# aaryaamoharir/ImageTransformations

Measured on AMD Instinct MI355X. Metric: Mpixels/sec, 5x5 Gaussian + bilinear rotate on 4K RGB; % HBM roofline, higher is better.
Workload: dtype u8/f32

## Files before the change

imagetransformations_amd/csrc/affine_route.h:

```cpp
#pragma once
#include "imgxf_common.h"
#include <algorithm>
#include <string.h>

namespace imgxf {

struct AffineParams {
    double m[6];
    int fx[6];
    int64_t q0, q3;
    int64_t q1, q4;
    int64_t x00, y00;
    u32 ntx_magic;
    int sx[4], sy[4];
    u8 fill[4];
    int xcd_regions;
};

constexpr int BILINEAR_LIST_MAX = 896;
struct TileList { int n; u32 idx[BILINEAR_LIST_MAX]; };

constexpr int MF_TILE_H = 64;
constexpr int WQ_PITCH = 28;
constexpr int WQ_MAXCH = 192;
constexpr int NQ_KW = 8;
constexpr int TALL_PITCH = 49, TALL_MAXROWS = 64;

struct AffineKnobs {
    bool fpb_set;
    int fpb;
    bool no_dma, no_lds, no_shear_fast, no_tall;
    int fpb_or(int dflt) const { return fpb_set ? fpb : dflt; }
};

enum AffineFamily {
    AF_GLOBAL,
    AF_BILINEAR_GLOBAL,
    AF_BILINEAR_LDS,
    AF_BILINEAR_INTERIOR,
    AF_BILINEAR_LIST,
    AF_BILINEAR_MF,
    AF_BILINEAR_WQ,
    AF_NEAREST_LDS,
    AF_NEAREST_DMA,
    AF_NEAREST_WQ,
    AF_SHEAR,
    AF_SHEAR_EDGES,
};

struct AffineLaunch {
    AffineFamily family;
    int c, filter, pitch, nbr, kw, tile_h;
    bool precise, dbg, dma, honly, defer;
    dim3 grid, block;
    size_t lds;
    int ntx, nty, fpb, nch, bh;
};

struct AffinePlan {
    AffineParams P;
    int n;
    AffineLaunch launch[2];
    TileList list;
};

inline int box_f64(double a, double b, int tw, int th, int extra) {
    return (int)ceil(fabs(a) * (tw - 1) + fabs(b) * (th - 1)) + extra;
}
inline int box_fx(int a, int b, int tw, int th, int extra) {
    return (int)ceil((fabs((double)a) * (tw - 1) + fabs((double)b) * (th - 1)) / 65536.0) + extra;
}
inline int packed_chunks(int bw) { return (bw * 3 + 15 + 15) / 16; }
inline bool aligned(const View& v, int bytes) {
    return ((((uintptr_t)v.p) | (uintptr_t)v.rs | (uintptr_t)v.fs) & (uintptr_t)(bytes - 1)) == 0;
}
inline bool offsets_fit_32(const View& v) { return (int64_t)v.h * v.rs < ((int64_t)1 << 32); }
inline u32 tile_magic(int ntx) { return (u32)((((uint64_t)1 << 32) + ntx - 1) / ntx); }
__host__ __device__ inline bool xcd_tile(unsigned b, int ntx, int nty, int regions, u32 magic, int& tx, int& ty) {
    const int T = ntx * nty, x = (int)(b & 7), l = (int)(b >> 3), q = T >> 3, r = T & 7;
    const int first = x * q + (x < r ? x : r), count = q + (x < r);
    if (l >= count) return false;
    if (!regions) {
        const int t = first + l;
        ty = magic ? (int)(((uint64_t)(u32)t * magic) >> 32) : t / ntx;
        tx = t - ty * ntx;
        return true;
    }
    const int last = first + count - 1;
    const int c0 = first / nty, r0 = first - c0 * nty, c1 = last / nty, r1 = last - c1 * nty;
    if (c1 == c0) { tx = c0; ty = r0 + l; return true; }
    const int whole = c1 - c0 - 1;
    const bool both = r0 <= r1 + 1;
    const int lo = both ? r0 : r1 + 1, hi = both ? r1 + 1 : r0;
    const int w1 = both ? whole + 2 : whole, n0 = lo * (whole + 1), n1 = (hi - lo) * w1;
    if (l < n0) { ty = l / (whole + 1); tx = c0 + 1 + (l - ty * (whole + 1)); }
    else if (l < n0 + n1) { const int k = l - n0, row = k / w1; ty = lo + row; tx = (both ? c0 : c0 + 1) + (k - row * w1); }
    else { const int k = l - n0 - n1, row = k / (whole + 1); ty = hi + row; tx = c0 + (k - row * (whole + 1)); }
    return true;
}
inline unsigned xcd_tile_grid(int ntx, int nty, int min_cols, AffineParams& P) {
    P.xcd_regions = ntx >= min_cols;
    return (unsigned)(ntx * nty);
}

inline AffineLaunch& add_launch(AffinePlan& R, AffineFamily family, dim3 grid, dim3 block, size_t lds) {
    AffineLaunch& L = R.launch[R.n++];
    L = AffineLaunch();
    L.family = family; L.grid = grid; L.block = block; L.lds = lds;
    return L;
}

inline bool plan_nearest_tiles(const View& s, const View& d, const AffineKnobs& K, AffinePlan& R) {
    AffineParams& P = R.P;
    bool nowrap = true;
    for (int cy = 0; cy < 2; ++cy)
        for (int cx = 0; cx < 2; ++cx) {
            const double X = cx ? d.w + 32 : 0, Y = cy ? d.h + 32 : 0;
            const double xs = (double)P.fx[2] + (double)P.fx[1] * Y + (double)P.fx[0] * X;
            const double ys = (double)P.fx[5] + (double)P.fx[4] * Y + (double)P.fx[3] * X;
            if (fabs(xs) > 2.0e9 || fabs(ys) > 2.0e9) nowrap = false;
        }
    const int bw = box_fx(P.fx[0], P.fx[1], 32, 32, 3), bh = box_fx(P.fx[3], P.fx[4], 32, 32, 3);
    const int ntx = (d.w + 31) / 32, nty = (d.h + 31) / 32;
    if (!(nowrap && bw <= 97 && bh <= 100 && (int64_t)ntx * nty < 0x7fffffff && d.n <= 65535)) return false;
    P.ntx_magic = tile_magic(ntx);
    {
        const int bwq = box_fx(P.fx[0], P.fx[1], 32, 16, 3), bhq = box_fx(P.fx[3], P.fx[4], 32, 16, 3);
        const int nchq = packed_chunks(bwq), kwq = (bhq * nchq + 63) / 64;
        const int ntxq = (d.w + 127) / 128, ntyq = (d.h + 15) / 16;
        if (aligned(s, 16) && aligned(d, 16) && (d.w * 3) % 16 == 0 && (s.w * 3) % 16 == 0 && s.w * 3 >= 16 && offsets_fit_32(s) &&
            offsets_fit_32(d) && !K.no_dma && kwq <= NQ_KW && (int64_t)ntxq * ntyq < ((int64_t)1 << 27)) {
            const int fpbq = std::max(1, std::min(K.fpb_or(1), d.n));
            const size_t nbufq = fpbq > 1 ? 2 : 1;
            AffineLaunch& L = add_launch(R, AF_NEAREST_WQ, dim3((unsigned)(ntxq * ntyq), (unsigned)((d.n + fpbq - 1) / fpbq)), dim3(256),
                                         nbufq * ((size_t)4 * ((size_t)bhq * nchq * 16 + 16) + 16 * 384));
            L.kw = kwq; L.ntx = ntxq; L.nty = ntyq; L.fpb = fpbq; L.nch = nchq; L.bh = bhq;
            return true;
        }
    }
    if (bw <= 49 && bh <= 52 && !K.no_dma && s.w * 3 >= 16 && (s.w * 3) % 16 == 0 && aligned(s, 16)) {
        const int bw64 = box_fx(P.fx[0], P.fx[1], 32, 64, 3), bh64 = box_fx(P.fx[3], P.fx[4], 32, 64, 3);
        if (bw64 <= 64 && bh64 <= 80 && !K.no_tall) {
            const int nty64 = (d.h + 63) / 64;
            const unsigned gx = xcd_tile_grid(ntx, nty64, 16, P);
            AffineLaunch& L = add_launch(R, AF_NEAREST_DMA, dim3(gx, (unsigned)d.n), dim3(256), (size_t)13 * 16 * bh64 + 32);
            L.tile_h = 64; L.ntx = ntx; L.nty = nty64;
        } else {
            AffineLaunch& L = add_launch(R, AF_NEAREST_DMA, dim3((unsigned)(ntx * nty), (unsigned)d.n), dim3(256), (size_t)11 * 16 * bh + 32);
            L.tile_h = 32; L.ntx = ntx; L.nty = nty;
        }
        return true;
    }
    const int pitch = bw <= 49 ? 49 : (bw <= 65 ? 65 : 97);
    AffineLaunch& L = add_launch(R, AF_NEAREST_LDS, dim3((unsigned)(ntx * nty), (unsigned)d.n), dim3(256), (size_t)pitch * bh * 4 + 16);
    L.pitch = pitch; L.ntx = ntx; L.nty = nty;
    return true;
}

inline bool plan_fixed_point(const View& d, const double* m, AffineParams& P) {
    bool fixed_ok = fabs(m[0]) < 64.0 && fabs(m[3]) < 64.0;
    for (int cy = 0; cy < 2 && fixed_ok; ++cy)
        for (int cx = 0; cx < 2; ++cx) {
            const double X = (cx ? d.w + 4 : 0) + 0.5, Y = (cy ? d.h : 0) + 0.5;
            const double xs = m[0] * X + m[1] * Y + m[2], ys = m[3] * X + m[4] * Y + m[5];
            if (!(fabs(xs) < 2097152.0 && fabs(ys) < 2097152.0)) fixed_ok = false;
        }
    P.q0 = fixed_ok ? llround(m[0] * 1099511627776.0) : 0;
    P.q3 = fixed_ok ? llround(m[3] * 1099511627776.0) : 0;
    fixed_ok = fixed_ok && fabs(m[1]) < 64.0 && fabs(m[4]) < 64.0;
    P.q1 = fixed_ok ? llround(m[1] * 1099511627776.0) : 0;
    P.q4 = fixed_ok ? llround(m[4] * 1099511627776.0) : 0;
    for (int k = 0; k < 4; ++k) {
        P.sx[k] = (int)((k * P.q0 + (k * P.q0 >= 0 ? 32768 : -32768)) / 65536);
        P.sy[k] = (int)((k * P.q3 + (k * P.q3 >= 0 ? 32768 : -32768)) / 65536);
    }
    if (fixed_ok) {
        const double x0d = (m[0] * 0.5 + m[1] * 0.5) + m[2] - 0.5, y0d = (m[3] * 0.5 + m[4] * 0.5) + m[5] - 0.5;
        P.x00 = (int64_t)floor(x0d * 1099511627776.0);
        P.y00 = (int64_t)floor(y0d * 1099511627776.0);
    }
    return fixed_ok;
}

inline bool plan_bilinear_tall(const View& s, const View& d, const double* m, int bw, int bh, int ntx, bool pr, bool want_f32,
                               const AffineKnobs& K, AffinePlan& R) {
    AffineParams& P = R.P;
    const int bwt = box_f64(m[0], m[1], 32, MF_TILE_H, 4), bht = box_f64(m[3], m[4], 32, MF_TILE_H, 4);
    const int ntyt = (d.h + MF_TILE_H - 1) / MF_TILE_H;
    if (bwt > TALL_PITCH || bht > TALL_MAXROWS || bw > TALL_PITCH || (int64_t)ntx * ntyt * ntx >= ((int64_t)1 << 32)) return false;
    const int fpb = K.fpb_or(16);
    const bool mf = !want_f32 && fpb >= 2 && d.n >= 2 && bht <= 64 && offsets_fit_32(d);
    if (mf && !K.no_dma) {
        const int bwq = box_f64(m[0], m[1], 32, 16, 4), bhq = box_f64(m[3], m[4], 32, 16, 4);
        const int nchq = packed_chunks(bwq);
        const int ntxq = (d.w + 127) / 128, ntyq = (d.h + 15) / 16;
        if (aligned(s, 16) && aligned(d, 16) && (d.w * 3) % 16 == 0 && s.w * 3 >= 16 &&
            bwq <= WQ_PITCH && bhq * nchq <= WQ_MAXCH && bhq * (WQ_PITCH / 4) <= 192 &&
            offsets_fit_32(s) && (int64_t)ntxq * ntyq < ((int64_t)1 << 27)) {
            const int fpbq = K.fpb_or(24);
            const unsigned gx = xcd_tile_grid(ntxq, ntyq, 8, P);
            AffineLaunch& L = add_launch(R, AF_BILINEAR_WQ, dim3(gx, (unsigned)((d.n + fpbq - 1) / fpbq)), dim3(256),
                                         (size_t)4 * ((size_t)bhq * WQ_PITCH * 4 + 2 * ((size_t)bhq * nchq * 16 + 64)) + 2 * 16 * 384);
            L.precise = pr; L.ntx = ntxq; L.nty = ntyq; L.fpb = fpbq; L.nch = nchq; L.bh = bhq;
            return true;
        }
    }
    const int nch = packed_chunks(bwt);
    if (mf && !K.no_dma && bht <= 52 && bwt <= 52 && 52 * nch <= 768 && aligned(s, 16) && s.w * 3 >= 16 && offsets_fit_32(s)) {
        const unsigned gx = xcd_tile_grid(ntx, ntyt, 16, P);
        AffineLaunch& L = add_launch(R, AF_BILINEAR_MF, dim3(gx, (unsigned)((d.n + fpb - 1) / fpb)), dim3(256),
                                     (size_t)52 * 56 * 4 + 2 * ((size_t)52 * nch * 16 + 64));
        L.precise = pr; L.pitch = 56; L.nbr = 13; L.dma = true; L.ntx = ntx; L.nty = ntyt; L.fpb = fpb; L.nch = nch;
        return true;
    }
    struct { int n; u32* idx; } list = {0, R.list.idx};
    const int64_t q0 = P.q0, q1 = P.q1, q3 = P.q3, q4 = P.q4, x00 = P.x00, y00 = P.y00;
    const int sw = s.w, sh = s.h, dw = d.w, dh = d.h;
    const int64_t ax = 31 * q0, bx = (MF_TILE_H - 1) * q1, ay = 31 * q3, by = (MF_TILE_H - 1) * q4;
    const int64_t xlo_o = std::min(ax, (int64_t)0) + std::min(bx, (int64_t)0), xhi_o = std::max(ax, (int64_t)0) + std::max(bx, (int64_t)0);
    const int64_t ylo_o = std::min(ay, (int64_t)0) + std::min(by, (int64_t)0), yhi_o = std::max(ay, (int64_t)0) + std::max(by, (int64_t)0);
    for (int ty = 0; ty < ntyt && list.n <= BILINEAR_LIST_MAX; ++ty)
        for (int tx = 0; tx < ntx; ++tx) {
            const int64_t XT = x00 + (int64_t)(tx * 32) * q0 + (int64_t)(ty * MF_TILE_H) * q1;
            const int64_t YT = y00 + (int64_t)(tx * 32) * q3 + (int64_t)(ty * MF_TILE_H) * q4;
            const bool clean = (int)((XT + xlo_o) >> 40) >= 0 && (int)((YT + ylo_o) >> 40) >= 0 &&
                               (int)((XT + xhi_o) >> 40) + 1 <= sw - 1 && (int)((YT + yhi_o) >> 40) + 1 <= sh - 1 &&
                               tx * 32 + 32 <= dw && ty * MF_TILE_H + MF_TILE_H <= dh &&
                               !((int)((XT + xhi_o) >> 40) + 1 == sw - 1 && (int)((YT + yhi_o) >> 40) + 1 == sh - 1);
            if (!clean) {
                if (list.n < BILINEAR_LIST_MAX) list.idx[list.n] = (u32)(ty * ntx + tx);
                ++list.n;
            }
        }
    R.list.n = list.n;
    if (list.n > BILINEAR_LIST_MAX) return false;
    if (list.n < ntx * ntyt && mf) {
        const int nbr = bht <= 52 ? 13 : 16;
        AffineLaunch& L = add_launch(R, AF_BILINEAR_MF, dim3((unsigned)(ntx * ntyt), (unsigned)((d.n + fpb - 1) / fpb)), dim3(256),
                                     (size_t)2 * TALL_PITCH * (4 * nbr) * 4 + 16);
        L.precise = pr; L.pitch = TALL_PITCH; L.nbr = nbr; L.ntx = ntx; L.nty = ntyt; L.fpb = fpb;
    } else if (list.n < ntx * ntyt) {
        AffineLaunch& L = add_launch(R, AF_BILINEAR_INTERIOR, dim3((unsigned)(ntx * ntyt), (unsigned)d.n), dim3(256),
                                     (size_t)TALL_PITCH * bht * 4 + 16);
        L.precise = pr; L.dbg = want_f32; L.pitch = TALL_PITCH; L.tile_h = MF_TILE_H; L.ntx = ntx; L.nty = ntyt;
    }
    if (list.n > 0) {
        AffineLaunch& L = add_launch(R, AF_BILINEAR_LIST, dim3((unsigned)((MF_TILE_H / 32) * list.n), (unsigned)d.n), dim3(256),
                                     (size_t)TALL_PITCH * bh * 4 + 16);
        L.precise = pr; L.dbg = want_f32; L.pitch = TALL_PITCH; L.tile_h = MF_TILE_H; L.ntx = ntx;
    }
    return true;
}

inline bool plan_bilinear_tiles(const View& s, const View& d, const double* m, bool pr, bool want_f32, const AffineKnobs& K,
                                AffinePlan& R) {
    const int bw = box_f64(m[0], m[1], 32, 32, 4), bh = box_f64(m[3], m[4], 32, 32, 4);
    const int ntx = (d.w + 31) / 32, nty = (d.h + 31) / 32;
    if (!(bw <= 97 && bh <= 100 && (int64_t)ntx * nty < 0x7fffffff && d.n <= 65535)) return false;
    R.P.ntx_magic = tile_magic(ntx);
    if (!K.no_tall && plan_bilinear_tall(s, d, m, bw, bh, ntx, pr, want_f32, K, R)) return true;
    const int pitch = bw <= 49 ? 49 : (bw <= 65 ? 65 : 97);
    AffineLaunch& L = add_launch(R, AF_BILINEAR_LDS, dim3((unsigned)(ntx * nty), (unsigned)d.n), dim3(256), (size_t)pitch * bh * 4 + 16);
    L.precise = pr; L.dbg = want_f32; L.pitch = pitch; L.ntx = ntx; L.nty = nty;
    return true;
}

inline bool horizontal_only(const double* m) {
    return m[3] == 0.0 && m[4] == 1.0 && m[5] == floor(m[5]) && fabs(m[5]) < 1.0e9;
}

inline int plan_affine(const View& s, const View& d, const double* m, int filter, bool precise, bool want_f32, const u8* fill,
                       const AffineKnobs& K, AffinePlan& R) {
    AffineParams& P = R.P;
    memset(&P, 0, sizeof(P));
    for (int i = 0; i < 6; ++i) P.m[i] = m[i];
    affine_fixed_matrix(m, P.fx);
    if (fill) for (int j = 0; j < d.c; ++j) P.fill[j] = fill[j];
    R.n = 0;
    R.list.n = 0;
    const bool pr = precise || filter == IMGXF_FILTER_NEAREST;
    if (filter == IMGXF_FILTER_NEAREST && s.c == 3 && !K.no_lds && aligned(s, 4) && plan_nearest_tiles(s, d, K, R)) return IMGXF_OK;
    const bool fixed_ok = plan_fixed_point(d, m, P);
    if (filter == IMGXF_FILTER_BILINEAR && (s.c == 1 || s.c == 3) && s.w >= 3 && s.h >= 2 && fixed_ok) {
        if (s.c == 3 && !K.no_lds && aligned(s, 4) && plan_bilinear_tiles(s, d, m, pr, want_f32, K, R)) return IMGXF_OK;
        constexpr int BW = 2 * 8 * 4, BH = (4 / 2) * (64 / 8);
        const int ntx = (d.w + BW - 1) / BW, nty = (d.h + BH - 1) / BH;
        const int64_t nb = (int64_t)ntx * nty * d.n;
        if (nb > 0x7fffffff) return IMGXF_ERR_SHAPE;
        AffineLaunch& L = add_launch(R, AF_BILINEAR_GLOBAL, dim3((unsigned)nb), dim3(256), 0);
        L.c = s.c; L.precise = pr; L.ntx = ntx; L.nty = nty;
        return IMGXF_OK;
    }
    const bool honly = horizontal_only(m);
    if (filter == IMGXF_FILTER_BICUBIC && honly && s.c == 3 && !want_f32 && !K.no_shear_fast && s.w >= 4) {
        AffineLaunch& L = add_launch(R, AF_SHEAR, dim3((unsigned)((d.w + 1023) / 1024), (unsigned)d.h, (unsigned)d.n), dim3(256), 0);
        L.precise = pr;
        L.defer = m[0] == 1.0;
        if (L.defer) add_launch(R, AF_SHEAR_EDGES, dim3((unsigned)((d.h * 8 + 255) / 256), (unsigned)d.n), dim3(256), 0);
        return IMGXF_OK;
    }
    AffineLaunch& L = add_launch(R, AF_GLOBAL, dim3((unsigned)((d.w + 255) / 256), (unsigned)((d.h + 3) / 4), (unsigned)d.n), dim3(64, 4), 0);
    L.c = s.c; L.filter = filter; L.precise = pr;
    L.honly = filter == IMGXF_FILTER_BICUBIC && honly;
    return IMGXF_OK;
}

}
```

imagetransformations_amd/csrc/affine_wq.inc:

```
#pragma once

namespace imgxf {


template <int OFF>
__device__ __forceinline__ u32 wq_bytes_at(const u32 (&q)[4]) {
    if constexpr ((OFF & 3) == 0) return q[OFF >> 2];
    else return __builtin_amdgcn_alignbyte(q[(OFF >> 2) + 1], q[OFF >> 2], (u32)(OFF & 3));
}

typedef u32 wq_u32x4 __attribute__((ext_vector_type(4)));

__device__ __forceinline__ void store16_sv(u8* base, u32 voff, wq_u32x4 o) {
    asm volatile("global_store_dwordx4 %0, %1, %2" : : "v"(voff), "v"(o), "s"(base) : "memory");
}

struct WqFlush {
    u32 rd[2], off[2];
    bool ok[2];
    __device__ __forceinline__ WqFlush(const View& d, const u32* slots, int lane, int wave, int txb, int sy0) {
        const int rb16 = (int)((int64_t)d.w * 3 / 16);
#pragma unroll
        for (int pass = 0; pass < 2; ++pass) {
            const int ch = pass * 64 + lane;
            const int r = wave * 4 + ch / 24, ck = ch - (ch / 24) * 24;
            ok[pass] = ch < 96 && sy0 + r < d.h && txb * 24 + ck < rb16;
            rd[pass] = (u32)(uintptr_t)(__attribute__((address_space(3))) const u32*)slots + (u32)((r * 96 + ck * 4) * 4);
            off[pass] = (u32)(sy0 + r) * (u32)d.rs + (u32)(txb * 384 + ck * 16);
        }
    }
    template <u32 SLOT_OFF>
    __device__ __forceinline__ void rows(u8* dframe) const {
#pragma unroll
        for (int pass = 0; pass < 2; ++pass) {
            if (ok[pass]) store16_sv(dframe, off[pass], *(const __attribute__((address_space(3))) wq_u32x4*)(uintptr_t)(rd[pass] + SLOT_OFF));
        }
    }
    __device__ __forceinline__ void operator()(u8* dframe, int par) const {
        if (par) rows<16 * 96 * 4>(dframe); else rows<0>(dframe);
    }
};

template <bool PRECISE>
__global__ __launch_bounds__(256, 3) void affine_bilinear_wq_kernel(View s, View d, AffineParams P, int ntx, int nty, int fpb,
                                                                   int nch, int rows) {
    constexpr int C = 3, SW = 32, BH = 16, BW = 4 * SW, PITCH = WQ_PITCH, NG = PITCH / 4;
    constexpr float GUARDP = 4.0f / 32768.0f;
    constexpr u32 GTOP = 8u << 17;
    constexpr int FONE = 1 << 24, FHALF = 1 << 23, CG32 = 1 << 6;
    extern __shared__ __attribute__((aligned(16))) u32 wq_lds[];
    int tyb, txb;
    if (!xcd_tile(blockIdx.x, ntx, nty, P.xcd_regions, 0, txb, tyb)) return;
    const int lane = threadIdx.x & 63, wave = __builtin_amdgcn_readfirstlane(threadIdx.x >> 6);
    const int f_begin = blockIdx.y * fpb, f_end = min(d.n, f_begin + fpb);
    const int sx0 = txb * BW + wave * SW, sy0 = tyb * BH;
    const bool wave_in = sx0 < d.w;

    const u32 pk_bytes = (u32)(rows * nch * 16 + 64);
    const u32 wave_bytes = (u32)(rows * PITCH * 4) + 2u * pk_bytes;
    u32* const srct = wq_lds + wave * (wave_bytes / 4);
    u32* const slots = wq_lds + 4 * (wave_bytes / 4);

    const int64_t XT = P.x00 + (int64_t)sx0 * P.q0 + (int64_t)sy0 * P.q1;
    const int64_t YT = P.y00 + (int64_t)sx0 * P.q3 + (int64_t)sy0 * P.q4;
    const int64_t ax = (SW - 1) * P.q0, bx = (BH - 1) * P.q1, ay = (SW - 1) * P.q3, by = (BH - 1) * P.q4;
    const int64_t xlo = XT + min(ax, (int64_t)0) + min(bx, (int64_t)0), xhi = XT + max(ax, (int64_t)0) + max(bx, (int64_t)0);
    const int64_t ylo = YT + min(ay, (int64_t)0) + min(by, (int64_t)0), yhi = YT + max(ay, (int64_t)0) + max(by, (int64_t)0);
    const int ux_lo = __builtin_amdgcn_readfirstlane((int)(xlo >> 40)), uy_lo = __builtin_amdgcn_readfirstlane((int)(ylo >> 40));
    const int sx_hi = __builtin_amdgcn_readfirstlane((int)(xhi >> 40) + 1), sy_hi = __builtin_amdgcn_readfirstlane((int)(yhi >> 40) + 1);
    const bool interior = ux_lo >= 0 && uy_lo >= 0 && sx_hi <= s.w - 1 && sy_hi <= s.h - 1 && sx0 + SW <= d.w && sy0 + BH <= d.h;

    const int lx = (lane & 7) * 4, x0 = sx0 + lx;
    u32 la[8];
    float w00[8], w01[8], w10[8], w11[8];
    u32 cneed = 0, fillm = 0, okm = 0;
#pragma unroll
    for (int half = 0; half < 2; ++half) {
        const int ly = half * 8 + (lane >> 3);
        const int64_t XL = XT + lx * P.q0 + ly * P.q1 - ((int64_t)ux_lo << 40);
        const int64_t YL = YT + lx * P.q3 + ly * P.q4 - ((int64_t)uy_lo << 40);
        const int Xb = (int)((XL + 32768) >> 16), Yb = (int)((YL + 32768) >> 16);
#pragma unroll
        for (int j = 0; j < 4; ++j) {
            const int k = half * 4 + j;
            const int X32 = Xb + P.sx[j], Y32 = Yb + P.sy[j];
            const u32 fx = (u32)X32 & (FONE - 1), fy = (u32)Y32 & (FONE - 1);
            const float dx = (float)fx * 5.9604644775390625e-08f, dy = (float)fy * 5.9604644775390625e-08f;
            const float ox = 1.0f - dx, oy = 1.0f - dy;
            w00[k] = ox * oy; w01[k] = dx * oy; w10[k] = ox * dy; w11[k] = dx * dy;
            la[k] = (u32)(((Y32 >> 24) * PITCH + (X32 >> 24)) * 4);
            const u32 gx = ((u32)X32 + CG32) & (FONE - 1), gy = ((u32)Y32 + CG32) & (FONE - 1);
            cneed |= (min(gx, gy) < 2u * CG32) ? 1u << k : 0u;
            if (!interior) {
                const int xi = (X32 >> 24) + ux_lo, yi = (Y32 >> 24) + uy_lo;
                const bool valid = x0 + j < d.w && sy0 + ly < d.h;
                const bool sure = (((fx & (FHALF - 1)) - CG32) < (u32)(FHALF - 2 * CG32)) &&
                                  (((fy & (FHALF - 1)) - CG32) < (u32)(FHALF - 2 * CG32));
                const bool inner = valid && sure && xi >= 0 && xi + 1 <= s.w - 1 && yi >= 0 && yi + 1 <= s.h - 1;
                const bool far_out = valid && sure && (xi < -1 || xi > s.w || yi < -1 || yi > s.h);
                if (!inner) { w00[k] = 0.0f; w01[k] = 0.0f; w10[k] = 0.0f; w11[k] = 0.0f; la[k] = 0u; }
                cneed = (cneed & ~(1u << k)) | ((valid && !inner && !far_out) ? 1u << k : 0u);
                fillm |= far_out ? 1u << k : 0u;
                okm |= valid ? 1u << k : 0u;
            }
        }
    }
    const bool fill_only = wave_in && !interior && __builtin_amdgcn_ballot_w64((okm & ~fillm) != 0u) == 0;
    const bool wave_on = wave_in && !fill_only;
    if (interior) okm = 0xffu;

    const int a0 = (ux_lo * 3) & ~15, e0 = ux_lo * 3 - a0;
    const u32 rgbx_bytes = (u32)(rows * PITCH * 4);
    const u32 pk_base = (u32)(uintptr_t)(__attribute__((address_space(3))) u32*)srct + rgbx_bytes;
    u32 dma_off[3];
    bool dma_ok[3];
    u32 ex_rd[3], ex_wr[3];
    bool ex_ok[3];
    {
        const u32 lim = (u32)(((int64_t)(s.h - 1) * s.rs + (int64_t)s.w * 3 - 16) & ~(int64_t)15);
#pragma unroll
        for (int i = 0; i < 3; ++i) {
            const int c = i * 64 + lane;
            const int row = c / nch, ch = c - row * nch;
            dma_ok[i] = c < rows * nch && wave_on;
            const int64_t go = (int64_t)clampi(uy_lo + row, 0, s.h - 1) * s.rs + a0 + 16 * ch;
            dma_off[i] = (u32)min(max(go, (int64_t)0), (int64_t)lim);
        }
#pragma unroll
        for (int it = 0; it < 3; ++it) {
            const int u = lane + 64 * it;
            const int rr = u / NG, t = u - rr * NG;
            ex_ok[it] = u < rows * NG;
            ex_rd[it] = pk_base + (u32)(rr * nch * 16 + ((e0 + 12 * t) & ~3));
            ex_wr[it] = pk_base - rgbx_bytes + (u32)((rr * PITCH + 4 * t) * 4);
            asm volatile("" : "+v"(ex_rd[it]), "+v"(ex_wr[it]));
        }
    }
    const int kw = (rows * nch + 63) / 64;
    auto dma_issue = [&](const u8* fb, int pbuf) {
#pragma unroll
        for (int i = 0; i < 3; ++i) {
            const u32 ldst = __builtin_amdgcn_readfirstlane(pk_base + (u32)pbuf * pk_bytes + (u32)(i * 1024));
            if (i < kw && dma_ok[i]) glds16_hidden(fb, dma_off[i], ldst);
        }
    };
    auto expand = [&](auto ph, int pbuf) {
        constexpr int PH = decltype(ph)::value;
        const u32 poff = (u32)pbuf * pk_bytes;
#pragma unroll
        for (int it = 0; it < 3; ++it) {
            if (!ex_ok[it]) continue;
            const __attribute__((address_space(3))) u32* q = (const __attribute__((address_space(3))) u32*)(uintptr_t)(ex_rd[it] + poff);
            const u32 dq[4] = {q[0], q[1], q[2], q[3]};
            const wq_u32x4 o = {wq_bytes_at<PH>(dq), wq_bytes_at<PH + 3>(dq), wq_bytes_at<PH + 6>(dq), wq_bytes_at<PH + 9>(dq)};
            *(__attribute__((address_space(3))) wq_u32x4*)(uintptr_t)ex_wr[it] = o;
        }
    };

    auto put_pixel = [&](u32 (&od)[2][3], int k, u32 val) {
        const int half = k >> 2, j = k & 3;
        u32 o0 = half ? od[1][0] : od[0][0], o1 = half ? od[1][1] : od[0][1], o2 = half ? od[1][2] : od[0][2];
        if (j == 0) o0 = (o0 & 0xff000000u) | val;
        else if (j == 1) { o0 = (o0 & 0x00ffffffu) | (val << 24); o1 = (o1 & 0xffff0000u) | (val >> 8); }
        else if (j == 2) { o1 = (o1 & 0x0000ffffu) | (val << 16); o2 = (o2 & 0xffffff00u) | (val >> 16); }
        else o2 = (o2 & 0x000000ffu) | (val << 8);
        if (half) { od[1][0] = o0; od[1][1] = o1; od[1][2] = o2; } else { od[0][0] = o0; od[0][1] = o1; od[0][2] = o2; }
    };

    auto slow_pixels = [&](u32 need, int f, u32 (&od)[2][3]) {
        const u8* sp = s.p + (int64_t)f * s.fs;
#pragma unroll 1
        for (u32 m = need; m; m &= m - 1) {
            const int k = __builtin_ctz(m), half = k >> 2, j = k & 3;
            const int y = sy0 + half * 8 + (lane >> 3);
            const bool unsure = (cneed >> k) & 1u;
            u32 val = 0;
            bool have = true;
            const double xc = (double)(x0 + j) + 0.5, yc = (double)y + 0.5;
            double xin = (P.m[0] * xc + P.m[1] * yc) + P.m[2];
            double yin = (P.m[3] * xc + P.m[4] * yc) + P.m[5];
            if (unsure && !(xin >= 0.0 && xin < (double)s.w && yin >= 0.0 && yin < (double)s.h)) {
                val = (u32)P.fill[0] | ((u32)P.fill[1] << 8) | ((u32)P.fill[2] << 16);
            } else {
                xin -= 0.5; yin -= 0.5;
                const double xfl = floor(xin), yfl = floor(yin);
                const int xq = (int)xfl, yq = (int)yfl;
                const double dxd = xin - xfl, dyd = yin - yfl;
                u32 p00, p01, p10, p11;
                if (unsure) {
                    const int xa = clampi(xq, 0, s.w - 1) * C, xb = clampi(xq + 1, 0, s.w - 1) * C;
                    const u8* r0 = sp + (int64_t)clampi(yq, 0, s.h - 1) * s.rs;
                    const bool has1 = (yq + 1 >= 0) && (yq + 1 < s.h);
                    const u8* r1 = has1 ? sp + (int64_t)(yq + 1) * s.rs : r0;
                    p00 = (u32)r0[xa] | ((u32)r0[xa + 1] << 8) | ((u32)r0[xa + 2] << 16);
                    p01 = (u32)r0[xb] | ((u32)r0[xb + 1] << 8) | ((u32)r0[xb + 2] << 16);
                    p10 = (u32)r1[xa] | ((u32)r1[xa + 1] << 8) | ((u32)r1[xa + 2] << 16);
                    p11 = (u32)r1[xb] | ((u32)r1[xb + 1] << 8) | ((u32)r1[xb + 2] << 16);
                } else {
                    const u32* tp = srct + (yq - uy_lo) * PITCH + (xq - ux_lo);
                    p00 = tp[0]; p01 = tp[1]; p10 = tp[PITCH]; p11 = tp[PITCH + 1];
                    have = (((p00 ^ p01) | (p10 ^ p11) | (p00 ^ p10)) << 8) != 0;
                }
#pragma unroll
                for (int c = 0; c < C; ++c) {
                    const double ta = (double)((p00 >> (8 * c)) & 0xffu), tb = (double)((p01 >> (8 * c)) & 0xffu);
                    const double tc = (double)((p10 >> (8 * c)) & 0xffu), te = (double)((p11 >> (8 * c)) & 0xffu);
                    const double w1 = ta + (tb - ta) * dxd, w2 = tc + (te - tc) * dxd;
                    const double w = w1 + (w2 - w1) * dyd;
                    val |= (u32)(u8)(int)w << (8 * c);
                }
            }
            if (have) put_pixel(od, k, val);
        }
    };

    auto gather_frame = [&](int f, u32* slot) {
        const u32 boff = (u32)(uintptr_t)(__attribute__((address_space(3))) const u32*)srct;
        u32 od[2][3] = {{0u, 0u, 0u}, {0u, 0u, 0u}};
        u32 need = cneed;
#pragma unroll
        for (int half = 0; half < 2; ++half) {
            if (half) __builtin_amdgcn_sched_barrier(0);
            u32 tq[4][3], mq[4];
#pragma unroll
            for (int j = 0; j < 4; ++j) {
                const int k = half * 4 + j;
                const u32* tp = (const u32*)(__attribute__((address_space(3))) const u32*)(uintptr_t)(boff + la[k]);
                const u32 p00 = tp[0], p01 = tp[1], p10 = tp[PITCH], p11 = tp[PITCH + 1];
                constexpr float X0 = PRECISE ? 256.0f + GUARDP : 0.0f;
                float v[3];
                v[0] = fmaf(w00[k], tapf<0>(p00), X0); v[1] = fmaf(w00[k], tapf<1>(p00), X0); v[2] = fmaf(w00[k], tapf<2>(p00), X0);
                v[0] = fmaf(w01[k], tapf<0>(p01), v[0]); v[1] = fmaf(w01[k], tapf<1>(p01), v[1]); v[2] = fmaf(w01[k], tapf<2>(p01), v[2]);
                v[0] = fmaf(w10[k], tapf<0>(p10), v[0]); v[1] = fmaf(w10[k], tapf<1>(p10), v[1]); v[2] = fmaf(w10[k], tapf<2>(p10), v[2]);
                v[0] = fmaf(w11[k], tapf<0>(p11), v[0]); v[1] = fmaf(w11[k], tapf<1>(p11), v[1]); v[2] = fmaf(w11[k], tapf<2>(p11), v[2]);
                if (PRECISE) {
#pragma unroll
                    for (int c = 0; c < 3; ++c) tq[j][c] = __builtin_amdgcn_alignbit(__float_as_uint(v[c]), __float_as_uint(v[c]), 15u);
                    mq[j] = min(min(tq[j][0], tq[j][1]), tq[j][2]);
                } else {
                    u32 (&o)[3] = od[half];
#pragma unroll
                    for (int c = 0; c < 3; ++c) {
                        const int bpos = j * 3 + c;
                        o[bpos >> 2] = __builtin_amdgcn_cvt_pk_u8_f32(floorf(v[c]), bpos & 3, o[bpos >> 2]);
                    }
                }
            }
            if (PRECISE) {
                constexpr u32 PAIR = 0x0c0c0400u, QUAD = 0x05040100u;
                const u32 a0 = __builtin_amdgcn_perm(tq[0][1], tq[0][0], PAIR), a1 = __builtin_amdgcn_perm(tq[1][0], tq[0][2], PAIR);
                const u32 a2 = __builtin_amdgcn_perm(tq[1][2], tq[1][1], PAIR), a3 = __builtin_amdgcn_perm(tq[2][1], tq[2][0], PAIR);
                const u32 a4 = __builtin_amdgcn_perm(tq[3][0], tq[2][2], PAIR), a5 = __builtin_amdgcn_perm(tq[3][2], tq[3][1], PAIR);
                od[half][0] = __builtin_amdgcn_perm(a1, a0, QUAD);
                od[half][1] = __builtin_amdgcn_perm(a3, a2, QUAD);
                od[half][2] = __builtin_amdgcn_perm(a5, a4, QUAD);
                const u32 mg = min(min(mq[0], mq[1]), min(mq[2], mq[3]));
                if (__builtin_amdgcn_ballot_w64(mg < GTOP) != 0) {
#pragma unroll
                    for (int j = 0; j < 4; ++j) need |= (mq[j] < GTOP) ? 1u << (half * 4 + j) : 0u;
                }
            }
        }
        need &= okm & ~fillm;
        if (need) slow_pixels(need, f, od);
        if (fillm && ((u32)P.fill[0] | (u32)P.fill[1] | (u32)P.fill[2])) {
            const u32 val = (u32)P.fill[0] | ((u32)P.fill[1] << 8) | ((u32)P.fill[2] << 16);
#pragma unroll 1
            for (u32 m = fillm; m; m &= m - 1) put_pixel(od, __builtin_ctz(m), val);
        }
#pragma unroll
        for (int half = 0; half < 2; ++half) {
            u32* ws = slot + (half * 8 + (lane >> 3)) * 96 + wave * 24 + (lane & 7) * 3;
            ws[0] = od[half][0]; ws[1] = od[half][1]; ws[2] = od[half][2];
        }
    };

    const WqFlush flush_slot(d, slots, lane, wave, txb, sy0);

    if (fill_only) {
        const u32 val = (u32)P.fill[0] | ((u32)P.fill[1] << 8) | ((u32)P.fill[2] << 16);
#pragma unroll
        for (int q = 0; q < 4; ++q) {
            u32* ws = slots + (q >> 1) * (16 * 96) + ((q & 1) * 8 + (lane >> 3)) * 96 + wave * 24 + (lane & 7) * 3;
            ws[0] = val | (val << 24); ws[1] = (val >> 8) | (val << 16); ws[2] = (val >> 16) | (val << 8);
        }
    }

    const u8* sdma = s.p + (int64_t)f_begin * s.fs;
    u8* dfl = d.p + (int64_t)f_begin * d.fs;
    if (wave_on) {
        dma_issue(sdma, 0); sdma += s.fs;
        if (f_begin + 1 < f_end) { dma_issue(sdma, 1); sdma += s.fs; }
    }
    const int ph = e0 & 3;
    int pb = 0;
#pragma unroll 1
    for (int f = f_begin; f < f_end; ++f) {
        const int par = (f - f_begin) & 1;
        if (wave_on) {
            if (f + 1 >= f_end) asm volatile("s_waitcnt vmcnt(0)" ::: "memory");
            else if (kw == 1) asm volatile("s_waitcnt vmcnt(1)" ::: "memory");
            else if (kw == 2) asm volatile("s_waitcnt vmcnt(2)" ::: "memory");
            else asm volatile("s_waitcnt vmcnt(3)" ::: "memory");
        }
        if (f > f_begin) { flush_slot(dfl, par ^ 1); dfl += d.fs; }
        if (wave_on) {
            if (ph == 0) expand(std::integral_constant<int, 0>(), pb);
            else if (ph == 1) expand(std::integral_constant<int, 1>(), pb);
            else if (ph == 2) expand(std::integral_constant<int, 2>(), pb);
            else expand(std::integral_constant<int, 3>(), pb);
            asm volatile("s_waitcnt lgkmcnt(0)" ::: "memory");
            if (f + 2 < f_end) { dma_issue(sdma, pb); sdma += s.fs; }
            gather_frame(f, slots + par * (16 * 96));
            pb ^= 1;
        }
        asm volatile("s_waitcnt lgkmcnt(0)\n\ts_barrier" ::: "memory");
    }
    flush_slot(dfl, (f_end - 1 - f_begin) & 1);
}


template <int KWT>
__device__ __forceinline__ void nq_wait() {
    static_assert(KWT >= 0 && KWT <= NQ_KW, "");
    if constexpr (KWT == 0) asm volatile("s_waitcnt vmcnt(0)" ::: "memory");
    else if constexpr (KWT == 1) asm volatile("s_waitcnt vmcnt(1)" ::: "memory");
    else if constexpr (KWT == 2) asm volatile("s_waitcnt vmcnt(2)" ::: "memory");
    else if constexpr (KWT == 3) asm volatile("s_waitcnt vmcnt(3)" ::: "memory");
    else if constexpr (KWT == 4) asm volatile("s_waitcnt vmcnt(4)" ::: "memory");
    else if constexpr (KWT == 5) asm volatile("s_waitcnt vmcnt(5)" ::: "memory");
    else if constexpr (KWT == 6) asm volatile("s_waitcnt vmcnt(6)" ::: "memory");
    else if constexpr (KWT == 7) asm volatile("s_waitcnt vmcnt(7)" ::: "memory");
    else asm volatile("s_waitcnt vmcnt(8)" ::: "memory");
}

template <int KW>
__global__ __launch_bounds__(256) void affine_nearest_wq_kernel(View s, View d, AffineParams P, int ntx, int nty, int fpb,
                                                                int nch, int rows) {
    constexpr int C = 3, SW = 32, BH = 16, BW = 4 * SW;
    extern __shared__ __attribute__((aligned(16))) u32 nq_lds[];
    int tyb, txb;
    if (!xcd_tile(blockIdx.x, ntx, nty, P.xcd_regions, 0, txb, tyb)) return;
    const int lane = threadIdx.x & 63, wave = __builtin_amdgcn_readfirstlane(threadIdx.x >> 6);
    const int f_begin = blockIdx.y * fpb, f_end = min(d.n, f_begin + fpb);
    const int sx0 = txb * BW + wave * SW, sy0 = tyb * BH;
    const int dpitch = nch * 16;
    const u32 box_bytes = (u32)(rows * dpitch + 16);
    const u32 nbuf = fpb > 1 ? 2u : 1u;
    char* const boxes = (char*)nq_lds + wave * (nbuf * box_bytes);
    u32* const slots = nq_lds + 4 * (nbuf * box_bytes) / 4;

    const int XT = P.fx[2] + P.fx[1] * sy0 + P.fx[0] * sx0;
    const int YT = P.fx[5] + P.fx[4] * sy0 + P.fx[3] * sx0;
    const int ax = (SW - 1) * P.fx[0], bx = (BH - 1) * P.fx[1], ay = (SW - 1) * P.fx[3], by = (BH - 1) * P.fx[4];
    const int sx_lo = max((XT + min(ax, 0) + min(bx, 0)) >> 16, 0), sx_hi = min((XT + max(ax, 0) + max(bx, 0)) >> 16, s.w - 1);
    const int sy_lo = max((YT + min(ay, 0) + min(by, 0)) >> 16, 0), sy_hi = min((YT + max(ay, 0) + max(by, 0)) >> 16, s.h - 1);
    const int bwc = sx_hi - sx_lo + 1, bhc = sy_hi - sy_lo + 1;
    const bool wave_in = sx0 < d.w && bwc > 0 && bhc > 0;
    const int a0 = (sx_lo * 3) & ~15;
    const int last_chunk = s.w * 3 - 16;

    const u32 fillw = (u32)P.fill[0] | ((u32)P.fill[1] << 8) | ((u32)P.fill[2] << 16);
    const int lx = (lane & 7) * 4;
    u32 bo[8];
    u32 inm = 0;
#pragma unroll
    for (int half = 0; half < 2; ++half) {
        const int ly = half * 8 + (lane >> 3);
        const int XL = XT + lx * P.fx[0] + ly * P.fx[1], YL = YT + lx * P.fx[3] + ly * P.fx[4];
#pragma unroll
        for (int j = 0; j < 4; ++j) {
            const int xi = ((XL + j * P.fx[0]) >> 16) - sx_lo, yi = ((YL + j * P.fx[3]) >> 16) - sy_lo;
            const bool in = wave_in && (u32)xi < (u32)bwc && (u32)yi < (u32)bhc;
            bo[half * 4 + j] = in ? (u32)(yi * dpitch + (xi + sx_lo) * 3 - a0) : 0u;
            inm |= in ? 1u << (half * 4 + j) : 0u;
        }
    }

    u32 dma_off[KW];
    bool dma_ok[KW];
#pragma unroll
    for (int i = 0; i < KW; ++i) {
        const int c = i * 64 + lane;
        const int row = c / nch, ch = c - row * nch;
        dma_ok[i] = wave_in && c < rows * nch;
        dma_off[i] = (u32)((int64_t)min(sy_lo + row, s.h - 1) * s.rs + min(a0 + ch * 16, last_chunk));
    }
    const u32 box_base = (u32)(uintptr_t)(__attribute__((address_space(3))) char*)boxes;
    auto dma_issue = [&](const u8* fb, int pbuf) {
#pragma unroll
        for (int i = 0; i < KW; ++i) {
            const u32 ldst = __builtin_amdgcn_readfirstlane(box_base + (u32)pbuf * box_bytes + (u32)(i * 1024));
            if (dma_ok[i]) glds16_hidden(fb, dma_off[i], ldst);
        }
    };
    auto gather_frame = [&](int pbuf, u32* slot) {
        const char* box = boxes + pbuf * box_bytes;
#pragma unroll
        for (int half = 0; half < 2; ++half) {
            u32 px[4];
#pragma unroll
            for (int j = 0; j < 4; ++j) {
                const int k = half * 4 + j;
                const u32* wp = (const u32*)(box + (bo[k] & ~3u));
                const u32 lo = wp[0], hi = wp[1];
                const u32 t = __builtin_amdgcn_alignbyte(hi, lo, bo[k] & 3u);
                px[j] = ((inm >> k) & 1u) ? (t & 0xffffffu) : fillw;
            }
            u32* ws = slot + (half * 8 + (lane >> 3)) * 96 + wave * 24 + (lane & 7) * 3;
            ws[0] = px[0] | (px[1] << 24);
            ws[1] = (px[1] >> 8) | (px[2] << 16);
            ws[2] = (px[2] >> 16) | (px[3] << 8);
        }
    };
    const WqFlush flush_slot(d, slots, lane, wave, txb, sy0);

    const u8* sdma = s.p + (int64_t)f_begin * s.fs;
    u8* dfl = d.p + (int64_t)f_begin * d.fs;
    dma_issue(sdma, 0); sdma += s.fs;
    if (f_begin + 1 < f_end) { dma_issue(sdma, 1); sdma += s.fs; }
#pragma unroll 1
    for (int f = f_begin; f < f_end; ++f) {
        const int it = f - f_begin;
        if (f + 1 >= f_end) nq_wait<0>(); else nq_wait<KW>();
        if (it) { flush_slot(dfl, (it - 1) & 1); dfl += d.fs; }
        gather_frame(it & 1, slots + (it & 1) * (16 * 96));
        asm volatile("s_waitcnt lgkmcnt(0)" ::: "memory");
        if (f + 2 < f_end) { dma_issue(sdma, it & 1); sdma += s.fs; }
        asm volatile("s_barrier" ::: "memory");
    }
    flush_slot(dfl, (f_end - 1 - f_begin) & 1);
}

}
```

Before: 389,100.

## Single-buffer packed DMA staging in WQ bilinear kernel to raise occupancy

Removes the double-buffered packed-source LDS staging in the wide-quad bilinear kernel, so only one frame's global-to-LDS copy is in flight and prefetch depth drops from two frames to one. This shrinks the LDS footprint per block, and the launch bound is raised from 3 to 5 blocks per CU so more blocks can be resident. The trade-off is less latency hiding inside each block: every frame now waits for all outstanding loads (vmcnt 0) before expanding, relying on extra resident blocks to cover memory latency. A compiler barrier on the flush-slot read addresses is also added to keep them in registers.

```diff
diff --git a/imagetransformations_amd/csrc/affine_route.h b/imagetransformations_amd/csrc/affine_route.h
--- a/imagetransformations_amd/csrc/affine_route.h
+++ b/imagetransformations_amd/csrc/affine_route.h
@@ -200,7 +200,7 @@
             const int fpbq = K.fpb_or(24);
             const unsigned gx = xcd_tile_grid(ntxq, ntyq, 8, P);
             AffineLaunch& L = add_launch(R, AF_BILINEAR_WQ, dim3(gx, (unsigned)((d.n + fpbq - 1) / fpbq)), dim3(256),
-                                         (size_t)4 * ((size_t)bhq * WQ_PITCH * 4 + 2 * ((size_t)bhq * nchq * 16 + 64)) + 2 * 16 * 384);
+                                         (size_t)4 * ((size_t)bhq * WQ_PITCH * 4 + (size_t)bhq * nchq * 16 + 64) + 2 * 16 * 384);
             L.precise = pr; L.ntx = ntxq; L.nty = ntyq; L.fpb = fpbq; L.nch = nchq; L.bh = bhq;
             return true;
         }
diff --git a/imagetransformations_amd/csrc/affine_wq.inc b/imagetransformations_amd/csrc/affine_wq.inc
--- a/imagetransformations_amd/csrc/affine_wq.inc
+++ b/imagetransformations_amd/csrc/affine_wq.inc
@@ -42,7 +42,7 @@
 };
 
 template <bool PRECISE>
-__global__ __launch_bounds__(256, 3) void affine_bilinear_wq_kernel(View s, View d, AffineParams P, int ntx, int nty, int fpb,
+__global__ __launch_bounds__(256, 5) void affine_bilinear_wq_kernel(View s, View d, AffineParams P, int ntx, int nty, int fpb,
                                                                    int nch, int rows) {
     constexpr int C = 3, SW = 32, BH = 16, BW = 4 * SW, PITCH = WQ_PITCH, NG = PITCH / 4;
     constexpr float GUARDP = 4.0f / 32768.0f;
@@ -57,7 +57,7 @@
     const bool wave_in = sx0 < d.w;
 
     const u32 pk_bytes = (u32)(rows * nch * 16 + 64);
-    const u32 wave_bytes = (u32)(rows * PITCH * 4) + 2u * pk_bytes;
+    const u32 wave_bytes = (u32)(rows * PITCH * 4) + pk_bytes;
     u32* const srct = wq_lds + wave * (wave_bytes / 4);
     u32* const slots = wq_lds + 4 * (wave_bytes / 4);
 
@@ -137,20 +137,19 @@
         }
     }
     const int kw = (rows * nch + 63) / 64;
-    auto dma_issue = [&](const u8* fb, int pbuf) {
+    auto dma_issue = [&](const u8* fb) {
 #pragma unroll
         for (int i = 0; i < 3; ++i) {
-            const u32 ldst = __builtin_amdgcn_readfirstlane(pk_base + (u32)pbuf * pk_bytes + (u32)(i * 1024));
+            const u32 ldst = __builtin_amdgcn_readfirstlane(pk_base + (u32)(i * 1024));
             if (i < kw && dma_ok[i]) glds16_hidden(fb, dma_off[i], ldst);
         }
     };
-    auto expand = [&](auto ph, int pbuf) {
+    auto expand = [&](auto ph) {
         constexpr int PH = decltype(ph)::value;
-        const u32 poff = (u32)pbuf * pk_bytes;
 #pragma unroll
         for (int it = 0; it < 3; ++it) {
             if (!ex_ok[it]) continue;
-            const __attribute__((address_space(3))) u32* q = (const __attribute__((address_space(3))) u32*)(uintptr_t)(ex_rd[it] + poff);
+            const __attribute__((address_space(3))) u32* q = (const __attribute__((address_space(3))) u32*)(uintptr_t)ex_rd[it];
             const u32 dq[4] = {q[0], q[1], q[2], q[3]};
             const wq_u32x4 o = {wq_bytes_at<PH>(dq), wq_bytes_at<PH + 3>(dq), wq_bytes_at<PH + 6>(dq), wq_bytes_at<PH + 9>(dq)};
             *(__attribute__((address_space(3))) wq_u32x4*)(uintptr_t)ex_wr[it] = o;
@@ -275,7 +274,8 @@
         }
     };
 
-    const WqFlush flush_slot(d, slots, lane, wave, txb, sy0);
+    WqFlush flush_slot(d, slots, lane, wave, txb, sy0);
+    asm volatile("" : "+v"(flush_slot.rd[0]), "+v"(flush_slot.rd[1]));
 
     if (fill_only) {
         const u32 val = (u32)P.fill[0] | ((u32)P.fill[1] << 8) | ((u32)P.fill[2] << 16);
@@ -288,31 +288,21 @@
 
     const u8* sdma = s.p + (int64_t)f_begin * s.fs;
     u8* dfl = d.p + (int64_t)f_begin * d.fs;
-    if (wave_on) {
-        dma_issue(sdma, 0); sdma += s.fs;
-        if (f_begin + 1 < f_end) { dma_issue(sdma, 1); sdma += s.fs; }
-    }
+    if (wave_on) { dma_issue(sdma); sdma += s.fs; }
     const int ph = e0 & 3;
-    int pb = 0;
 #pragma unroll 1
     for (int f = f_begin; f < f_end; ++f) {
         const int par = (f - f_begin) & 1;
-        if (wave_on) {
-            if (f + 1 >= f_end) asm volatile("s_waitcnt vmcnt(0)" ::: "memory");
-            else if (kw == 1) asm volatile("s_waitcnt vmcnt(1)" ::: "memory");
-            else if (kw == 2) asm volatile("s_waitcnt vmcnt(2)" ::: "memory");
-            else asm volatile("s_waitcnt vmcnt(3)" ::: "memory");
-        }
+        if (wave_on) asm volatile("s_waitcnt vmcnt(0)" ::: "memory");
         if (f > f_begin) { flush_slot(dfl, par ^ 1); dfl += d.fs; }
         if (wave_on) {
-            if (ph == 0) expand(std::integral_constant<int, 0>(), pb);
-            else if (ph == 1) expand(std::integral_constant<int, 1>(), pb);
-            else if (ph == 2) expand(std::integral_constant<int, 2>(), pb);
-            else expand(std::integral_constant<int, 3>(), pb);
+            if (ph == 0) expand(std::integral_constant<int, 0>());
+            else if (ph == 1) expand(std::integral_constant<int, 1>());
+            else if (ph == 2) expand(std::integral_constant<int, 2>());
+            else expand(std::integral_constant<int, 3>());
             asm volatile("s_waitcnt lgkmcnt(0)" ::: "memory");
-            if (f + 2 < f_end) { dma_issue(sdma, pb); sdma += s.fs; }
+            if (f + 1 < f_end) { dma_issue(sdma); sdma += s.fs; }
             gather_frame(f, slots + par * (16 * 96));
-            pb ^= 1;
         }
         asm volatile("s_waitcnt lgkmcnt(0)\n\ts_barrier" ::: "memory");
     }
```

Result: faster. 411,100, median of 6 (+5.7%).
